# OpenPPL/ppq

Hardware: AMD Instinct MI355X
Metric: calibration samples/sec (RuntimeCalibrationPass, KL 2048-bin, ResNet-50 INT8) (higher is better)
Workload: dtype f32; 1 GPU; ResNet-50 topology (53 Conv + 1 Gemm, BN folded, seeded He init), RuntimeCalibrationPass kl 2048 bins, per-tensor INT8 activations, per-channel INT8 weights, 279 batches x 32 x 3x224x224 per GPU; samples=8928, batch=32, observed_tensors=72, rccl_ranks=1, async_observe=False, cache_params=False, channels_last=False, fuse_params=True, batch_observations=True, reuse_activations=False, replayed_batches=0, hip_graph=auto, graph_replays=0, miopen_find=False

## Files before the change

include/ppq_hip.h:

```cpp
#ifndef PPQ_HIP_H_
#define PPQ_HIP_H_

#include <stdint.h>

#ifdef __cplusplus
extern "C" {
#endif

typedef enum {
    PPQHIP_OK = 0,
    PPQHIP_ERR_INVALID_VALUE = -1,
    PPQHIP_ERR_UNSUPPORTED = -2,
    PPQHIP_ERR_HIP = -3
} ppqhip_status;

#define PPQHIP_ABI_VERSION 4

const char* ppqhip_last_error(void);
int ppqhip_version(void);
int ppqhip_device_arch(char* buf, int n);

int ppqhip_fq_linear_t(const float* x, const float* scale, const float* offset, float* out,
                       int64_t n, int clip_min, int clip_max, int rounding, void* stream);

// ... 368 lines not shown

enum { PPQHIP_MXFP8_E4M3 = 0, PPQHIP_MXFP8_E5M2 = 1, PPQHIP_MXFP6_E3M2 = 2, PPQHIP_MXFP6_E2M3 = 3, PPQHIP_MXFP4_E2M1 = 4,
       PPQHIP_MXINT8 = 5 };
int ppqhip_mx_fq(const float* x, float* y, uint8_t* scale_codes, int64_t outer, int64_t axis_len, int64_t inner, int format,
                 void* stream);
typedef struct ppqhip_mx_job {
    const float* x;
    float* y;
    uint8_t* scale_codes;
    int64_t outer, axis_len, inner;
    int32_t format, reserved;
} ppqhip_mx_job;
int ppqhip_mx_fq_multi(const ppqhip_mx_job* jobs, int num_jobs, void* stream);

int ppqhip_mx_pack(const float* x, uint8_t* elements, uint8_t* scales, int64_t outer, int64_t axis_len, int64_t inner, int format,
                   void* stream);
typedef struct ppqhip_mx_pack_job {
    const float* x;
    uint8_t* elements;
    uint8_t* scales;
    int64_t outer, axis_len, inner;
    int32_t format, reserved;
} ppqhip_mx_pack_job;
int ppqhip_mx_pack_multi(const ppqhip_mx_pack_job* jobs, int num_jobs, void* stream);
int ppqhip_mx_unpack(const uint8_t* elements, const uint8_t* scales, float* y, int64_t outer, int64_t axis_len, int64_t inner,
                     int format, void* stream);
typedef struct ppqhip_mx_unpack_job {
    const uint8_t* elements;
    const uint8_t* scales;
    float* y;
    int64_t outer, axis_len, inner;
    int32_t format, reserved;
} ppqhip_mx_unpack_job;
int ppqhip_mx_unpack_multi(const ppqhip_mx_unpack_job* jobs, int num_jobs, void* stream);

int ppqhip_mx_gemm(const uint8_t* a_elements, const uint8_t* a_scales, int a_format, const uint8_t* b_elements,
                   const uint8_t* b_scales, int b_format, const float* bias, float* c, int64_t m, int64_t n, int64_t k,
                   void* stream);

int ppqhip_mx_conv2d(const uint8_t* x_elements, const uint8_t* x_scales, int x_format, const uint8_t* w_elements,
                     const uint8_t* w_scales, int w_format, const float* bias, float* y, int64_t n, int64_t c, int64_t h, int64_t w,
                     int64_t o, int64_t kh, int64_t kw, int64_t stride_h, int64_t stride_w, int64_t pad_h, int64_t pad_w,
                     int64_t dil_h, int64_t dil_w, void* stream);

int ppqhip_mx_gemm_fused(const uint8_t* a_elements, const uint8_t* a_scales, int a_format, const uint8_t* b_elements,
                         const uint8_t* b_scales, int b_format, const float* bias, const float* residual, int relu, float* c,
                         uint8_t* out_elements, uint8_t* out_scales, int out_format, int64_t m, int64_t n, int64_t k, void* stream);
int ppqhip_mx_conv2d_fused(const uint8_t* x_elements, const uint8_t* x_scales, int x_format, const uint8_t* w_elements,
                           const uint8_t* w_scales, int w_format, const float* bias, const float* residual, int relu, float* y,
                           uint8_t* out_elements, uint8_t* out_scales, int out_format, int64_t n, int64_t c, int64_t h, int64_t w,
                           int64_t o, int64_t kh, int64_t kw, int64_t stride_h, int64_t stride_w, int64_t pad_h, int64_t pad_w,
                           int64_t dil_h, int64_t dil_w, void* stream);

#define PPQHIP_PROF_MAX_KERNELS 48
typedef struct {
    char name[48];
    int64_t launches;
    double total_ms;
    double total_bytes;
} ppqhip_prof_entry;
int ppqhip_prof_enable(int on);
int ppqhip_prof_collect(ppqhip_prof_entry* entries, int max_entries);
double ppqhip_prof_event_overhead_us(void* stream, int pairs);

#ifdef __cplusplus
}
#endif
#endif
```

ppq_amd/_lib.py:

```python
import ctypes
import os

_HERE = os.path.dirname(os.path.abspath(__file__))
LIB_PATH = os.path.join(_HERE, 'libppq_hip.so')

c_f32p = ctypes.c_void_p
c_i32p = ctypes.c_void_p
c_f64p = ctypes.c_void_p
c_i64 = ctypes.c_int64
c_int = ctypes.c_int
c_flt = ctypes.c_float
c_vp = ctypes.c_void_p

ABI_VERSION = 4


NOT_FUSED = 1


class ProfEntry(ctypes.Structure):
    _fields_ = [('name', ctypes.c_char * 48), ('launches', ctypes.c_int64),
                ('total_ms', ctypes.c_double), ('total_bytes', ctypes.c_double)]


# ... 55 lines not shown
    'ppqhip_fq_float_multi_table_bytes': (c_i64, [c_int]),
    'ppqhip_fq_float_multi': (c_int, [c_vp, c_int, c_int, c_vp, c_int, c_vp]),
    'ppqhip_quantile_multi_workspace_bytes': (c_i64, [c_int, c_i64]),
    'ppqhip_quantile_t_multi': (c_int, [c_vp, c_int, c_flt, c_vp, c_vp]),
    'ppqhip_quantile_debug_layout': (None, [c_vp]),
    'ppqhip_quantile_hot_layout': (None, [c_vp]),
    'ppqhip_minmax_t_slots_multi': (c_int, [c_vp, c_int, c_vp]),
    'ppqhip_hist_t_rows_multi': (c_int, [c_vp, c_int, c_int, c_int, c_i64, c_vp]),
    'ppqhip_channel_sum': (c_int, [c_f32p, c_i64, c_i64, c_i64, c_f64p, c_vp]),
    'ppqhip_hist_rows': (c_i64, []),
    'ppqhip_hist_sym_t_rows': (c_int, [c_f32p, c_i64, c_flt, c_int, c_i32p, c_i64, c_vp]),
    'ppqhip_hist_asym_t_rows': (c_int, [c_f32p, c_i64, c_flt, c_flt, c_int, c_i32p, c_i64, c_vp]),
    'ppqhip_hist_rows_finish': (c_int, [c_i32p, c_i64, c_i32p, c_vp]),
    'ppqhip_check_bin_rule': (c_int, [c_f32p, c_i64, c_flt, c_flt, c_int, c_vp, c_vp]),
    'ppqhip_minmax_slots': (c_i64, []),
    'ppqhip_minmax_t_slots': (c_int, [c_f32p, c_i64, c_f32p, c_vp]),
    'ppqhip_minmax_slots_finish': (c_int, [c_f32p, c_f32p, c_vp]),
    'ppqhip_mse_loss_host': (c_flt, [ctypes.POINTER(ctypes.c_int64), c_i64, c_int, c_int, c_int]),
    'ppqhip_mse_search_workspace_bytes': (c_i64, [c_i64]),
    'ppqhip_mse_search': (c_int, [c_i32p, c_i64, c_i64, c_f64p, c_f64p, c_int, c_int, c_int, c_i32p, c_vp, c_vp]),
    'ppqhip_kl_num_candidates': (c_i64, [c_i64, c_int]),
    'ppqhip_kl_losses': (c_int, [c_i32p, c_i64, c_i64, c_int, c_f64p, c_vp]),
    'ppqhip_tensor_clip_t': (c_int, [c_f32p, c_f32p, c_f32p, c_f32p, c_i64, c_vp]),
    'ppqhip_tensor_clip_c': (c_int, [c_f32p, c_f32p, c_f32p, c_f32p, c_i64, c_i64, c_i64, c_vp]),
    'ppqhip_rounding_loss': (c_int, [c_f32p, c_f32p, c_f32p, c_f32p, c_i64, c_i64, c_i64, c_int, c_int, c_int, c_vp]),
    'ppqhip_rounding_loss_bwd': (c_int, [c_f32p, c_f32p, c_f32p, c_f32p, c_f32p, c_i64, c_i64, c_i64, c_int, c_int,
                                         c_int, c_vp]),
    'ppqhip_adaround_fwd_multi': (c_int, [c_vp, c_int, c_vp]),
    'ppqhip_adaround_bwd_multi': (c_int, [c_vp, c_int, c_f32p, c_vp]),
    'ppqhip_roundtune_fwd_multi': (c_int, [c_vp, c_int, c_vp]),
    'ppqhip_equalize_scale_multi': (c_int, [c_vp, c_int, c_vp]),
    'ppqhip_equalize_apply_multi': (c_int, [c_vp, c_int, c_vp]),
    'ppqhip_split_plan_multi': (c_int, [c_vp, c_int, c_vp]),
    'ppqhip_split_apply_multi': (c_int, [c_vp, c_int, c_vp]),
    'ppqhip_ssd_scales_multi': (c_int, [c_vp, c_int, c_vp]),
    'ppqhip_ssd_apply_multi': (c_int, [c_vp, c_int, c_vp]),
    'ppqhip_fq_measure_rows_multi': (c_int, [c_vp, c_int, c_vp]),
    'ppqhip_fetch_rows_multi': (c_int, [c_vp, c_int, c_vp]),
    'ppqhip_measure_rows_multi': (c_int, [c_vp, c_int, c_vp]),
    'ppqhip_measure_finish_multi': (c_int, [c_vp, c_int, c_vp]),
    'ppqhip_stat_moments_multi': (c_int, [c_vp, c_int, c_vp]),
    'ppqhip_stat_shape_multi': (c_int, [c_vp, c_int, c_vp]),
    'ppqhip_mx_fq': (c_int, [c_f32p, c_f32p, c_vp, c_i64, c_i64, c_i64, c_int, c_vp]),
    'ppqhip_mx_fq_multi': (c_int, [c_vp, c_int, c_vp]),
    'ppqhip_mx_pack': (c_int, [c_f32p, c_vp, c_vp, c_i64, c_i64, c_i64, c_int, c_vp]),
    'ppqhip_mx_pack_multi': (c_int, [c_vp, c_int, c_vp]),
    'ppqhip_mx_unpack': (c_int, [c_vp, c_vp, c_f32p, c_i64, c_i64, c_i64, c_int, c_vp]),
    'ppqhip_mx_unpack_multi': (c_int, [c_vp, c_int, c_vp]),
    'ppqhip_mx_gemm': (c_int, [c_vp, c_vp, c_int, c_vp, c_vp, c_int, c_f32p, c_f32p, c_i64, c_i64, c_i64, c_vp]),
    'ppqhip_prof_enable': (c_int, [c_int]),
    'ppqhip_mx_conv2d': (c_int, [c_vp, c_vp, c_int, c_vp, c_vp, c_int, c_f32p, c_f32p] + [c_i64] * 13 + [c_vp]),
    'ppqhip_mx_gemm_fused': (c_int, [c_vp, c_vp, c_int, c_vp, c_vp, c_int, c_f32p, c_f32p, c_int, c_f32p, c_vp, c_vp, c_int, c_i64, c_i64, c_i64, c_vp]),
    'ppqhip_mx_conv2d_fused': (c_int, [c_vp, c_vp, c_int, c_vp, c_vp, c_int, c_f32p, c_f32p, c_int, c_f32p, c_vp, c_vp, c_int] + [c_i64] * 13 + [c_vp]),
    'ppqhip_prof_collect': (c_int, [ctypes.POINTER(ProfEntry), c_int]),
    'ppqhip_prof_event_overhead_us': (ctypes.c_double, [c_vp, c_int]),
}

if not os.path.exists(LIB_PATH):
    raise ImportError(
        f'{LIB_PATH} is missing: the HIP kernel library has not been built.  Run '
        '`python -c "import __graft_entry__ as g; g.build()"` or `make -C ppq_amd/csrc` (needs hipcc, '
        'targets gfx950).  ppq_amd has no CPU / PyTorch fallback by design.')

import torch

_torch_hip = os.path.join(os.path.dirname(torch.__file__), 'lib', 'libamdhip64.so')
if os.path.exists(_torch_hip):
    ctypes.CDLL(_torch_hip, mode=ctypes.RTLD_GLOBAL)

try:
    lib = ctypes.CDLL(LIB_PATH)
except OSError as e:
    raise ImportError(f'cannot load {LIB_PATH}: {e}') from e

for _name, (_res, _args) in PROTOTYPES.items():
    _fn = getattr(lib, _name)
    _fn.restype = _res
    _fn.argtypes = _args


if lib.ppqhip_version() != ABI_VERSION:
    raise ImportError(f'{LIB_PATH} has ABI version {lib.ppqhip_version()}, this package needs {ABI_VERSION}: rebuild it '
                      '(`make -C ppq_amd/csrc` or `python -c "import __graft_entry__ as g; g.build()"`)')


def last_error() -> str:
    msg = lib.ppqhip_last_error()
    return msg.decode('utf-8', 'replace') if msg else ''
```

ppq_amd/ffi.py:

```python
import math
import threading
import weakref
from typing import List

import numpy as np
import torch

from . import _lib
from ._lib import lib

_KERNEL_FAILURE = 'Kernel Failure, '


_raw_stream = torch._C._cuda_getCurrentRawStream
_get_device = torch._C._cuda_getDevice


def _stream() -> int:
    return _raw_stream(_get_device())


def _check(t: torch.Tensor, dtype: torch.dtype, name: str) -> None:
    if not isinstance(t, torch.Tensor):
        raise TypeError(f'{name}: expected a torch.Tensor, got {type(t)}')
# ... 124 lines not shown
_HIST_JOB = np.dtype([('x', '<u8'), ('rows', '<u8'), ('n', '<i8'), ('p0', '<f4'), ('p1', '<f4')])


def _epilogue_geometry(ts, bias_list):
    t0 = ts[0]
    if not isinstance(t0, torch.Tensor) or t0.dtype is not _F32 or not t0.is_cuda or t0.dim() != 4 or t0.numel() == 0:
        return None
    shape, strides, dev = t0.shape, t0.stride(), t0.device
    for t in ts[1:]:
        if not isinstance(t, torch.Tensor) or t.dtype is not _F32 or t.device != dev or t.shape != shape or t.stride() != strides:
            return None
    C = int(shape[1])
    for bias in bias_list:
        if (not isinstance(bias, torch.Tensor) or bias.dtype is not _F32 or bias.device != dev or bias.dim() != 1
                or bias.numel() != C or not bias.is_contiguous()):
            return None
    if t0.is_contiguous(): return C, int(shape[2]) * int(shape[3])
    if t0.is_contiguous(memory_format=torch.channels_last): return C, 1
    return None


def _pool_launch(y: torch.Tensor, geo, pool):
    k, s, p = (int(v) for v in pool)
    if geo is None or not y.is_contiguous() or k < 1 or s < 1 or p < 0: return None
    N, C, H, W = (int(v) for v in y.shape)
    if H + 2 * p < k or W + 2 * p < k: return None
    pooled = torch.empty((N, C, (H + 2 * p - k) // s + 1, (W + 2 * p - k) // s + 1), dtype=_F32, device=y.device)
    return pooled, (y.numel(), C, H, W), (k, s, p, 1, 0)


def bias_act_(y: torch.Tensor, bias: torch.Tensor, relu: bool, pool=None):
    geo = _epilogue_geometry([y], [bias])
    if pool is not None:
        args = _pool_launch(y, geo, pool)
        if args is None: return None
        with _DeviceOf(y):
            ok = _fused_or_raise(lib.ppqhip_bias_act_pool(y.data_ptr(), bias.data_ptr(), args[0].data_ptr(), *args[1],
                                                          1 if relu else 0, *args[2], _stream()))
        return args[0] if ok else None
    if geo is None: return False
    with _DeviceOf(y):
        _raise(lib.ppqhip_bias_act(y.data_ptr(), bias.data_ptr(), y.numel(), geo[0], geo[1], 1 if relu else 0, _stream()))
    return True


def bias_add_act(a: torch.Tensor, bias_a: torch.Tensor, b: torch.Tensor, bias_b, relu: bool):
    geo = _epilogue_geometry([a, b], [bias_a] if bias_b is None else [bias_a, bias_b])
    if geo is None or a.data_ptr() == b.data_ptr(): return None
    out = torch.empty_like(a)
    with _DeviceOf(a):
        _raise(lib.ppqhip_bias_add_act(a.data_ptr(), bias_a.data_ptr(), b.data_ptr(), 0 if bias_b is None else bias_b.data_ptr(),
                                       out.data_ptr(), a.numel(), geo[0], geo[1], 1 if relu else 0, _stream()))
    return out


def _sink_slots(job, dev) -> int:
    if job is None: return 0
    slots = job[1]
    if (job[0] != 'minmax' or slots.dtype is not _F32 or slots.device != dev or not slots.is_contiguous()
            or slots.numel() != 2 * lib.ppqhip_minmax_slots()): raise ValueError('no sink for this job')
    return slots.data_ptr()


def _fused_or_raise(status: int) -> bool:
    if status == _lib.NOT_FUSED: return False
    _raise(status)
    return True


def bias_act_stats_(y: torch.Tensor, bias: torch.Tensor, relu: bool, job, pool=None, store: bool = True):
    geo = _epilogue_geometry([y], [bias])
    if geo is None or job is None: return None if pool is not None else False
    try: slots = _sink_slots(job, y.device)
    except ValueError: return None if pool is not None else False
    if pool is not None:
        args = _pool_launch(y, geo, pool)
        if args is None: return None
        with _DeviceOf(y):
            ok = _fused_or_raise(lib.ppqhip_bias_act_pool_stats(y.data_ptr(), bias.data_ptr(), args[0].data_ptr(), *args[1],
                                                                1 if relu else 0, *args[2], slots, 1 if store else 0, _stream()))
        return args[0] if ok else None
    with _DeviceOf(y):
        return _fused_or_raise(lib.ppqhip_bias_act_stats(y.data_ptr(), bias.data_ptr(), y.numel(), geo[0], geo[1],
                                                         1 if relu else 0, slots, _stream()))


ELIDE_A, ELIDE_B = 1, 2


def bias_add_act_stats(a: torch.Tensor, bias_a: torch.Tensor, b: torch.Tensor, bias_b, relu: bool, job_a, job_b, job_out,
                       elide: int = 0):
    geo = _epilogue_geometry([a, b], [bias_a] if bias_b is None else [bias_a, bias_b])
    if geo is None or a.data_ptr() == b.data_ptr(): return None
    if bias_b is None and job_b is not None: return None
    try: slots = [_sink_slots(j, a.device) for j in (job_a, job_b, job_out)]
    except ValueError: return None
    if not any(slots): return None
    out = torch.empty_like(a)
    args = (a.data_ptr(), bias_a.data_ptr(), b.data_ptr(), 0 if bias_b is None else bias_b.data_ptr(), out.data_ptr(),
            a.numel(), geo[0], geo[1], 1 if relu else 0, slots[0], slots[1], slots[2])
    with _DeviceOf(a):
        if elide: ok = _fused_or_raise(lib.ppqhip_bias_add_act_stats2(*args, int(elide), _stream()))
        else: ok = _fused_or_raise(lib.ppqhip_bias_add_act_stats(*args, _stream()))
    return out if ok else None


# ... 1778 lines not shown
```

ppq_amd/harness.py:

```python
import contextlib
from typing import Callable, Dict, List, Optional

import torch
import torch.nn.functional as F

from .core import LinearQuantizationConfig, QuantizationStates, TensorQuantizationConfig, is_initial
from .core import QuantizationProperty as P
from .qfunction import PPQuantFunction

PASSIVE_OPERATIONS = {'MaxPool', 'GlobalMaxPool', 'Reshape', 'Flatten', 'Identity', 'Dropout', 'Slice', 'Pad', 'Resize',
                      'Split', 'Transpose', 'Interp', 'Squeeze', 'Unsqueeze'}
COMPUTING_OP = {'Conv', 'Gemm', 'ConvTranspose', 'MatMul'}


class Variable:
    def __init__(self, name: str, value: torch.Tensor = None, is_parameter: bool = False):
        self.name = name
        self.value = value
        self.stored_value = None
        self.is_parameter = is_parameter
        self.dest_ops: List['Operation'] = []
        self.source_op: Optional['Operation'] = None

    def __hash__(self): return hash(self.name)
# ... 43 lines not shown
        return list(zip(self.config.input_quantization_config, self.inputs)) + \
            list(zip(self.config.output_quantization_config, self.outputs))

    def dequantize(self):
        if getattr(self, '_dequantized', False): return self
        for cfg, _ in self.config_with_variable:
            cfg.detail['Stored State'] = cfg.state
            cfg.state = QuantizationStates.FP32
        self._swap_parameters()
        self._dequantized = True
        return self

    def restore_quantize_state(self):
        if not getattr(self, '_dequantized', False): return self
        for cfg, _ in self.config_with_variable:
            if 'Stored State' in cfg.detail: cfg.state = cfg.detail.pop('Stored State')
        self._swap_parameters()
        self._dequantized = False
        return self

    def baking_parameters(self, quant_func: Callable):
        for config, var in self.config_with_variable:
            if var.is_parameter and QuantizationStates.is_activated(config.state):
                var.value = quant_func(var.value, config)
                config.state = (QuantizationStates.BAKED if config.state == QuantizationStates.ACTIVATED
                                else QuantizationStates.PASSIVE_BAKED)


class BaseGraph:
    def __init__(self, name: str):
        self.name = name
        self.operations: Dict[str, Operation] = {}
        self.variables: Dict[str, Variable] = {}
        self.inputs: Dict[str, Variable] = {}
        self.outputs: Dict[str, Variable] = {}

    def create_variable(self, name: str, value=None, is_parameter=False) -> Variable:
        v = Variable(name, value, is_parameter)
        self.variables[name] = v
        return v

    def create_operation(self, op_type: str, name: str, inputs: List[Variable], attributes: dict = None) -> Variable:
        out = self.create_variable(name + '_out')
        op = Operation(name, op_type, attributes, list(inputs), [out])
        out.source_op = op
        for v in inputs: v.dest_ops.append(op)
        self.operations[name] = op
        return out

    def topological_sort(self) -> List[Operation]:
        return list(self.operations.values())


def _forward(op: Operation, x: List[torch.Tensor]):
    t, a = op.type, op.attributes
    if t == 'Conv':
        return F.conv2d(x[0], x[1], x[2] if len(x) > 2 else None, stride=a.get('strides', 1),
                        padding=a.get('pads', 0), groups=a.get('group', 1))
    if t == 'Gemm': return F.linear(x[0], x[1], x[2] if len(x) > 2 else None)
    if t == 'MatMul': return torch.matmul(x[0], x[1])
    if t == 'Relu': return F.relu(x[0])
    if t == 'Gelu': return F.gelu(x[0])
    if t == 'Add': return x[0] + x[1]
    if t == 'MaxPool': return F.max_pool2d(x[0], a['kernel_shape'], a.get('strides', 1), a.get('pads', 0))
    if t == 'GlobalAveragePool': return F.adaptive_avg_pool2d(x[0], 1)
    if t == 'Flatten': return torch.flatten(x[0], 1)
    if t == 'LayerNormalization': return F.layer_norm(x[0], x[0].shape[-1:], x[1], x[2])
    if t == 'Softmax': return F.softmax(x[0], dim=a.get('axis', -1))
    if t == 'Mul': return x[0] * (x[1] if len(x) > 1 else a['value'])
    if t == 'Reshape': return x[0].reshape(a['shape'])
    if t == 'Transpose': return x[0].permute(a['perm'])
    if t == 'Concat': return torch.cat([v.expand(x[-1].shape[0], *v.shape[1:]) if v.shape[0] == 1 else v for v in x],
                                       dim=a.get('axis', 1))
    if t == 'Slice': return x[0].narrow(a['axis'], a['start'], a['length'])
    if t == 'Resize': return F.interpolate(x[0], scale_factor=a.get('scale', 2), mode=a.get('mode', 'nearest'))
    raise NotImplementedError(f'Graph op: {op.name}({op.type}) has no backend implementation')


class EpilogueGroup:
    __slots__ = ('kind', 'ops', 'convs', 'add', 'relu', 'keep', 'pool')

    def __init__(self, kind, ops, convs, add, relu, keep=(), pool=None):
        self.kind, self.ops, self.convs, self.add, self.relu, self.keep = kind, ops, convs, add, relu, frozenset(keep)
        self.pool = pool

    def __repr__(self): return f'{self.kind}({", ".join(op.name for op in self.ops)})'


def pool_window(op: Operation) -> Optional[tuple]:
    a = op.attributes

    def square(value):
        if isinstance(value, (list, tuple)):
            if not 1 <= len(value) <= 2 or any(v != value[0] for v in value): return None
            value = value[0]
        return value if isinstance(value, int) and not isinstance(value, bool) else None
    if 'kernel_shape' not in a or square(a.get('dilations', 1)) != 1 or a.get('ceil_mode', 0) not in (0, False): return None
    window = tuple(square(v) for v in (a['kernel_shape'], a.get('strides', 1), a.get('pads', 0)))
    return None if any(v is None for v in window) else window


def _in_cfg(op, i):
    return op.config.input_quantization_config[i] if isinstance(op, QuantableOperation) else None


def _out_cfg(op, i):
    return op.config.output_quantization_config[i] if isinstance(op, QuantableOperation) else None


def plan_epilogues(operations: List[Operation], hooks: Dict[str, object] = None, keep=(), passes_through: Callable = None,
                   grad_enabled: bool = False) -> List[EpilogueGroup]:
# ... 70 lines not shown
        return EpilogueGroup('P1', [conv, relu] + ([pool] if pool is not None else []), [conv], None, relu, keep, pool)

    groups, i = [], 0
    while i < len(operations):
        g = try_p2(i) if operations[i].type == 'Conv' else None
        if g is None and operations[i].type == 'Conv': g = try_p1(i)
        if g is None:
            i += 1
            continue
        groups.append(g)
        i += len(g.ops)
    return groups


def elidable_stores(grp: EpilogueGroup, hooks, jobs: Dict[str, tuple], recorder=None) -> set:
    if recorder is not None or not hooks: return set()
    if grp.kind == 'P2': producers, reader = grp.convs, grp.add
    elif grp.pool is not None: producers, reader = [grp.relu], grp.pool
    else: return set()
    reader_hook = hooks.get(reader.name)
    out = set()
    for op in producers:
        v, hook = op.outputs[0], hooks.get(op.name)
        if len(v.dest_ops) != 1 or v.dest_ops[0] is not reader or v.name in grp.keep: continue
        if op.name not in jobs or hook is None or not isinstance(op, QuantableOperation): continue
        obs = [hook._observer_table.get(c) for c in op.config.output_quantization_config]
        if len(obs) != 1 or obs[0] is None or not obs[0].reads_only_its_job(): continue
        if reader_hook is not None and isinstance(reader, QuantableOperation) and any(
                c in reader_hook._observer_table for x, c in zip(reader.inputs, reader.config.input_quantization_config) if x is v):
            continue
        out.add(op.name)
    return out


class TorchExecutor:
    def __init__(self, graph: BaseGraph, device: str = 'cuda'):
        self._graph = graph
        self._device = device
        self._default_quant_fn = PPQuantFunction
        self.cache_parameter_quantization = False
        self._param_cache: Dict[str, tuple] = {}
        self.fuse_parameter_quantization = True
        self._plans: list = []
        self._plan_signature = None
        self._plan_cache: Dict[tuple, list] = {}
        self._fused: Dict[tuple, torch.Tensor] = {}
        self._delegates: Dict[object, Callable] = {}
        self._overrides: Dict[str, Callable] = {}
        self._takes_packed: set = set()
        self._group_overrides: Dict[str, tuple] = {}
        self.fuse_epilogues = True
        self._epilogue_cache: Dict[tuple, dict] = {}
        self.channels_last = False
        for v in graph.variables.values():
            if v.is_parameter and v.value is not None: v.value = v.value.to(device)

    def use_channels_last(self) -> 'TorchExecutor':
        self.channels_last = True
        for v in self._graph.variables.values():
            if v.is_parameter and isinstance(v.value, torch.Tensor) and v.value.dim() == 4:
                v.value = v.value.contiguous(memory_format=torch.channels_last)
        return self

    def _place(self, value: torch.Tensor) -> torch.Tensor:
        value = value.to(self._device)
        if self.channels_last and value.dim() == 4: value = value.contiguous(memory_format=torch.channels_last)
        return value

    def register_quantize_delegate(self, config, delegator: Callable) -> None:
        self._delegates[config] = delegator

    def remove_quantize_delegate(self, config) -> None:
        self._delegates.pop(config, None)

    def register_operation_override(self, op_name: str, fn: Callable, takes_packed: bool = False) -> None:
        if op_name not in self._graph.operations: raise KeyError(f'register_operation_override: the graph has no operation {op_name!r}')
        if not callable(fn): raise TypeError(f'register_operation_override: fn must be callable, got {type(fn)}')
        self._overrides[op_name] = fn
        if takes_packed: self._takes_packed.add(op_name)
        else: self._takes_packed.discard(op_name)

    def remove_operation_override(self, op_name: str) -> None:
        self._overrides.pop(op_name, None)
        self._takes_packed.discard(op_name)

    def register_group_override(self, op_names: List[str], fn: Callable) -> None:
        if not op_names: raise ValueError('register_group_override: no operations')
        for name in op_names:
            if name not in self._graph.operations: raise KeyError(f'register_group_override: the graph has no operation {name!r}')
        if not callable(fn): raise TypeError(f'register_group_override: fn must be callable, got {type(fn)}')
        self._group_overrides[op_names[0]] = (tuple(op_names), fn)

    def remove_group_override(self, first_name: str) -> None:
        self._group_overrides.pop(first_name, None)

    def _group_plan(self, operations: List[Operation], hooks, output_names, all_float: bool) -> Dict[str, tuple]:
        if not self._group_overrides: return {}
        hooks = hooks or {}
        keep = set(self._graph.outputs) | set(output_names or ())
        at = {op.name: i for i, op in enumerate(operations)}
        plan = {}
        for first, (names, fn) in self._group_overrides.items():
            if any(n not in at or n in hooks for n in names): continue
            if any(at[a] >= at[b] for a, b in zip(names, names[1:])): continue
            ops = [operations[at[n]] for n in names]
            if any(v.name in keep for m in ops[:-1] for v in m.outputs): continue
            need = set()
            for v in ops[-1].outputs:
                handed = [d.name in self._takes_packed and d.name in self._overrides and d.name not in hooks and d.name in at
                          and d.inputs[0] is v and sum(1 for x in d.inputs if x is v) == 1 for d in v.dest_ops]
                if all_float or v.name in keep or not handed or not all(handed): need.add(v.name)
            plan[first] = (ops, fn, need)
        return plan

    def _run_group(self, entry: tuple, raw_of: Callable, packed: Dict[str, object]) -> Dict[str, object]:
        ops, fn, need = entry
        inside = {v.name for m in ops for v in m.outputs}
        inputs = [[None if v.name in inside else raw_of(v) for v in m.inputs] for m in ops]
        head = ops[0]
        if head.name in self._takes_packed and head.inputs[0].name in packed: inputs[0][0] = packed[head.inputs[0].name]
        if any(x is None for k, m in enumerate(ops) for x, v in zip(inputs[k], m.inputs) if v.name not in inside):
            raise ValueError(f'group override of {head.name}: an input was not computed')
        values, handed = fn(ops, inputs, need)
        out = {}
        for m in ops:
            for v in m.outputs:
                if v.name in values: out[v.name] = values[v.name]
                elif v.name in handed and v.name not in need: out[v.name] = handed[v.name]
                else: raise RuntimeError(f'group override of {head.name}: no {"float " if v.name in need else ""}value for {v.name}')
        packed.update(handed)
        return out

    def _override_inputs(self, op: Operation, raw_in: list, packed: Dict[str, object]) -> list:
        if packed and op.name in self._takes_packed and op.inputs[0].name in packed:
            raw_in = list(raw_in)
            raw_in[0] = packed[op.inputs[0].name]
        return raw_in

    def quantize_function(self, tensor: torch.Tensor, config=None) -> torch.Tensor:
        if self._delegates and config in self._delegates:
            return self._delegates[config](tensor, config)
        return self._default_quant_fn(tensor, config)

    def _input_side(self, op: Operation, raw_in: list, hook) -> list:
        qin, cfgs = raw_in, None
        if isinstance(op, QuantableOperation):
            cfgs = list(op.config.input_quantization_config)
            qin = [self._quantize_parameter(v, c) if v.is_parameter else self.quantize_function(x, c)
                   for v, x, c in zip(op.inputs, raw_in, cfgs)]
        if hook is not None: qin = hook.pre_forward_hook(inputs=raw_in, quant_inputs=qin, quant_configs=cfgs)
        return qin

    def _output_side(self, op: Operation, outs, hook) -> list:
        fp_outs = outs = list(outs) if isinstance(outs, (list, tuple)) else [outs]
        cfgs = None
        if isinstance(op, QuantableOperation):
            cfgs = list(op.config.output_quantization_config)
            outs = [self.quantize_function(y, c) for y, c in zip(outs, cfgs)]
        if hook is not None: outs = hook.post_forward_hook(outputs=fp_outs, quant_outputs=outs, quant_configs=cfgs)
        return outs

    def _step(self, op: Operation, raw_in: list, hook, packed: Optional[Dict[str, object]]) -> list:
        override = self._overrides.get(op.name) if hook is None else None
        if override is not None: outs = override(op, self._override_inputs(op, raw_in, packed))
        else: outs = _forward(op, self._input_side(op, raw_in, hook))
        return self._output_side(op, outs, hook)

    def _walk(self, operations: List[Operation], hooks, output_names: List[str], read: Callable, write: Callable,
              hand_packed: bool = False, write_aliases: bool = True, done: Callable = None, unfed: str = None) -> None:
        groups, packed = self._group_plan(operations, hooks, output_names, not hand_packed), {}
        plan = self._epilogue_plan(operations, hooks, output_names, [m.name for e in groups.values() for m in e[0]])
        fused_done = set()
        for op in operations:
            if op.name in fused_done: continue
            vals = None
            if op.name in groups:
                members = groups[op.name][0]
                vals, aliases = self._run_group(groups[op.name], read, packed), members[:-1]
            elif op.name in plan:
                grp = plan[op.name]
                vals, members, aliases = self._run_epilogue(grp, read, hooks), grp.ops, (grp.add or grp.convs[0],)
            if vals is None:
                raw_in = [read(v) for v in op.inputs]
                if unfed and any(x is None for x in raw_in): raise ValueError(f'{unfed}: input of {op.name} was not fed')
                write(op, self._step(op, raw_in, hooks.get(op.name) if hooks else None, packed if hand_packed else None))
            else:
                for m in members:
                    fused_done.add(m.name)
                    if write_aliases or m not in aliases: write(m, [vals[v.name] for v in m.outputs])
            if done is not None and done(): break

    def forward_with_gradient(self, inputs, output_names: List[str] = None, hooks=None):
        return TorchExecutor.forward.__wrapped__(self, inputs, output_names, hooks)

    def partial_graph_forward(self, operations: List[Operation], feed_dict: Dict[str, torch.Tensor],
                              output_names: List[str], with_gradient: bool = False) -> List[torch.Tensor]:
        g = self._graph
        results = [None] * len(output_names)

        def write(op, outs):
            for v, y in zip(op.outputs, outs):
                v.value = y
                if v.name in output_names: results[output_names.index(v.name)] = y
        with contextlib.nullcontext() if with_gradient else torch.no_grad():
            for name, value in feed_dict.items(): g.variables[name].value = self._place(value)
            self._fused_parameters(operations)
            self._walk(operations, None, output_names, lambda v: v.value, write, unfed='partial_graph_forward')
        for v in g.variables.values():
            if not v.is_parameter: v.value = None
        return results

    def _fused_parameters(self, operations=None) -> None:
        self._fused = {}
        if not self.fuse_parameter_quantization or self._default_quant_fn is not PPQuantFunction: return
        from .ffi import FloatingQuantizePlan, LinearQuantizePlan
        todo, sig = [], []
        for op in (self._graph.operations.values() if operations is None else operations):
            if not isinstance(op, QuantableOperation): continue
# ... 27 lines not shown
                if floating:
                    plan = FloatingQuantizePlan([(v.value, c.scale, c.offset, axis, c.exponent_bits, c.mantissa_bits,
                                                  c.quant_min, c.quant_max) for v, c, axis, _, _ in items], rounding=rnd)
                else:
                    plan = LinearQuantizePlan([(v.value, c.scale, c.offset, axis, c.quant_min, c.quant_max)
                                               for v, c, axis, _, _ in items], rounding=rnd)
                self._plans.append((plan, [(v.name, id(c)) for v, c, _, _, _ in items]))
            self._plan_signature = sig
            if len(self._plan_cache) >= 8: self._plan_cache.pop(next(iter(self._plan_cache)))
            self._plan_cache[tuple(sig)] = self._plans
        for plan, keys in self._plans:
            for key, out in zip(keys, plan.run()): self._fused[key] = out

    def _epilogue_plan(self, operations: List[Operation], hooks, output_names, grouped=()) -> Dict[str, EpilogueGroup]:
        if not self.fuse_epilogues or torch.is_grad_enabled() or self._default_quant_fn is not PPQuantFunction: return {}
        states = tuple(c.state for op in operations if isinstance(op, QuantableOperation)
                       for c in (*op.config.input_quantization_config, *op.config.output_quantization_config))
        sig = (tuple(op.name for op in operations), tuple((k, id(h)) for k, h in hooks.items()) if hooks else (),
               tuple(output_names or ()), tuple(id(c) for c in self._delegates), states, tuple(sorted(self._overrides)), tuple(sorted(grouped)))
        plan = self._epilogue_cache.get(sig)
        if plan is None:
            delegates = self._delegates

            def passes_through(c): return not QuantizationStates.is_activated(c.state) and c not in delegates
            groups = plan_epilogues(operations, hooks, set(self._graph.outputs) | set(output_names or ()), passes_through)
            if self._overrides:
                groups = [g for g in groups if not any(m.name in self._overrides and not (hooks and m.name in hooks) for m in g.ops)]
            if grouped:
                groups = [g for g in groups if not any(m.name in grouped for m in g.ops)]
            plan = {g.ops[0].name: g for g in groups}
            if len(self._epilogue_cache) >= 8: self._epilogue_cache.pop(next(iter(self._epilogue_cache)))
            self._epilogue_cache[sig] = plan
        return plan

    def _run_epilogue(self, grp: EpilogueGroup, raw_of: Callable, hooks) -> Optional[Dict[str, torch.Tensor]]:
        from .ffi import (ELIDE_A, ELIDE_B, bias_act_, bias_act_hist_, bias_act_stats_, bias_add_act, bias_add_act_hist,
                          bias_add_act_stats)
        for conv in grp.convs:
            x, w = raw_of(conv.inputs[0]), conv.inputs[1].value
            if not (isinstance(x, torch.Tensor) and x.is_cuda and x.dtype == torch.float32 and x.dim() == 4
                    and isinstance(w, torch.Tensor) and w.dim() == 4): return None
            fmt = torch.channels_last if self.channels_last else torch.contiguous_format
            if not (x.is_contiguous(memory_format=fmt) and w.is_contiguous(memory_format=fmt)): return None
        if grp.add is not None:
            b_var = grp.add.inputs[1]
            if b_var.source_op not in grp.convs:
                b = raw_of(b_var)
                if not (isinstance(b, torch.Tensor) and b.is_cuda and b.dtype == torch.float32): return None
        hooks = hooks or {}
        ys, biases = {}, {}
        for conv in grp.ops[:len(grp.convs)]:
            qin = self._input_side(conv, [raw_of(v) for v in conv.inputs], hooks.get(conv.name))
            a = conv.attributes
            ys[conv.name] = F.conv2d(qin[0], qin[1], None, stride=a.get('strides', 1), padding=a.get('pads', 0),
                                     groups=a.get('group', 1))
            biases[conv.name] = qin[2]
        if grp.kind == 'P1':
            conv = grp.convs[0]
            y = ys[conv.name]
            stored = {grp.relu.name: y}
            fed = self._epilogue_sinks(grp, hooks, stored, y)
            window = pool_window(grp.pool) if grp.pool is not None and not self.channels_last else None
            pooled, elided = None, set()
            if fed is not None:
                job = fed[0].get(grp.relu.name)
                launch = bias_act_hist_ if job is not None and job[0] == 'hist_rows' else bias_act_stats_
                if window is not None:
                    elided = elidable_stores(grp, hooks, fed[0], fed[1].recorder)
                    pooled = launch(y, biases[conv.name], True, job, pool=window, store=not elided)
                    if pooled is None: elided = set()
                if pooled is None and not launch(y, biases[conv.name], True, job): fed = None
            if fed is None:
                if window is not None: pooled = bias_act_(y, biases[conv.name], relu=True, pool=window)
                if pooled is None and not bias_act_(y, biases[conv.name], relu=True):
                    y.add_(biases[conv.name].view(1, -1, 1, 1)).relu_()
            tail = {conv.name: y, grp.relu.name: y}
            if grp.pool is not None: tail[grp.pool.name] = pooled
        else:
            conv_a = grp.convs[0]
            a = ys[conv_a.name]
            conv_b = grp.convs[1] if len(grp.convs) > 1 else None
            b = ys[conv_b.name] if conv_b is not None else raw_of(grp.add.inputs[1])
            bias_b = biases[conv_b.name] if conv_b is not None else None
            stored = {conv_a.name: a, grp.relu.name: None}
            if conv_b is not None: stored[conv_b.name] = b
            fed, out, elided = self._epilogue_sinks(grp, hooks, stored, a), None, set()
            if fed is not None:
                jobs = fed[0]
                elided = elidable_stores(grp, hooks, jobs, fed[1].recorder)
                mask = (ELIDE_A if conv_a.name in elided else 0) | (ELIDE_B if conv_b is not None and conv_b.name in elided else 0)
                launch = bias_add_act_hist if next(iter(jobs.values()))[0] == 'hist_rows' else bias_add_act_stats
                out = launch(a, biases[conv_a.name], b, bias_b, True, jobs.get(conv_a.name),
                             jobs.get(conv_b.name) if conv_b is not None else None, jobs.get(grp.relu.name), mask)
                if out is None: fed, elided = None, set()
                else: stored[grp.relu.name] = out
            if out is None: out = bias_add_act(a, biases[conv_a.name], b, bias_b, relu=True)
            if out is None:
                a.add_(biases[conv_a.name].view(1, -1, 1, 1))
                if conv_b is not None: b.add_(biases[conv_b.name].view(1, -1, 1, 1))
                out = F.relu(a + b)
            tail = {conv_a.name: a, grp.add.name: out, grp.relu.name: out}
            if conv_b is not None: tail[conv_b.name] = b
        if fed is not None:
            for name, job in fed[0].items(): fed[1].prepay(stored[name], job[1])
        values: Dict[str, torch.Tensor] = {}
        for op in grp.ops:
            hook = hooks.get(op.name)
            if op.type != 'Conv':
# ... 374 lines not shown
```

Before: 3858 samples/s.

## Add native MFMA 1x1 conv kernel and route selected pointwise convs to it

```diff
diff --git a/include/ppq_hip.h b/include/ppq_hip.h
--- a/include/ppq_hip.h
+++ b/include/ppq_hip.h
@@ -444,6 +444,9 @@
                            int64_t o, int64_t kh, int64_t kw, int64_t stride_h, int64_t stride_w, int64_t pad_h, int64_t pad_w,
                            int64_t dil_h, int64_t dil_w, void* stream);
 
+int ppqhip_conv1x1(const float* x, const float* w, const float* bias, float* y, int64_t n, int64_t c, int64_t h, int64_t wd,
+                   int64_t o, int64_t stride, void* stream);
+
 #define PPQHIP_PROF_MAX_KERNELS 48
 typedef struct {
     char name[48];
diff --git a/ppq_amd/_lib.py b/ppq_amd/_lib.py
--- a/ppq_amd/_lib.py
+++ b/ppq_amd/_lib.py
@@ -131,7 +131,8 @@
     'ppqhip_mx_conv2d': (c_int, [c_vp, c_vp, c_int, c_vp, c_vp, c_int, c_f32p, c_f32p] + [c_i64] * 13 + [c_vp]),
     'ppqhip_mx_gemm_fused': (c_int, [c_vp, c_vp, c_int, c_vp, c_vp, c_int, c_f32p, c_f32p, c_int, c_f32p, c_vp, c_vp, c_int, c_i64, c_i64, c_i64, c_vp]),
     'ppqhip_mx_conv2d_fused': (c_int, [c_vp, c_vp, c_int, c_vp, c_vp, c_int, c_f32p, c_f32p, c_int, c_f32p, c_vp, c_vp, c_int] + [c_i64] * 13 + [c_vp]),
-    'ppqhip_prof_collect': (c_int, [ctypes.POINTER(ProfEntry), c_int]),
+    'ppqhip_conv1x1': (c_int, [c_f32p, c_f32p, c_f32p, c_f32p, c_i64, c_i64, c_i64, c_i64, c_i64, c_i64, c_vp]),
+    'ppqhip_prof_collect':(c_int, [ctypes.POINTER(ProfEntry), c_int]),
     'ppqhip_prof_event_overhead_us': (ctypes.c_double, [c_vp, c_int]),
 }
 
diff --git a/ppq_amd/csrc/pointwise_conv.hip b/ppq_amd/csrc/pointwise_conv.hip
--- /dev/null
+++ b/ppq_amd/csrc/pointwise_conv.hip
@@ -0,0 +1,194 @@
+#include "common.hpp"
+#include "job_table.hpp"
+
+namespace ppqhip {
+namespace {
+
+typedef float f32x16 __attribute__((ext_vector_type(16)));
+
+struct PwArgs {
+    const float* x; const float* w; const float* bias; float* y;
+    uint32_t c, o, q;
+    uint32_t in_plane, out_plane;
+    uint32_t in_w, stride;
+    uint32_t tiles_m;
+    FastDiv div_plane, div_wo, div_tiles_m;
+};
+
+template <int WM, int WN, int TM, int TN, int BK, bool VEC>
+__global__ __launch_bounds__(256) void conv1x1_kernel(const PwArgs g) {
+    static_assert(WM * WN == 4 && (BK == 16 || BK == 32), "4 waves; BK 16 or 32");
+    constexpr int BM = WM * TM * 32, BN = WN * TN * 32, RS = BK + 4, HK = BK / 2, LW = VEC ? 4 : 1;
+    constexpr int WL = BM * BK / (256 * LW), XL = BK * BN / (256 * LW);
+    constexpr int WROWS = 256 * LW / BK, XROWS = 256 * LW / BN;
+    static_assert(BN / LW <= 256 && WL >= 1 && XL >= 1, "tile too small / too wide for the loader");
+    typedef float ldv __attribute__((ext_vector_type(LW)));
+    __shared__ __attribute__((aligned(16))) float Ws[2][BM * RS];
+    __shared__ __attribute__((aligned(16))) float Xs[2][BK * BN];
+
+    const uint32_t t = threadIdx.x, lane = t & 63u, wave = t >> 6;
+    const uint32_t tq = fdiv(blockIdx.x, g.div_tiles_m), tm = blockIdx.x - tq * g.tiles_m;
+    const uint32_t m0 = tm * BM, q0 = tq * BN;
+
+    const uint32_t wk = (t % (BK / LW)) * LW, wm = t / (BK / LW);
+    const uint32_t xc = (t % (BN / LW)) * LW, xk = t / (BN / LW);
+    uint32_t woff[WL], xoff;
+#pragma unroll
+    for (int r = 0; r < WL; r++) woff[r] = min(m0 + wm + WROWS * r, g.o - 1u) * g.c + wk;
+    {
+        const uint32_t qx = min(q0 + xc, g.q - LW);
+        const uint32_t img = fdiv(qx, g.div_plane), p = qx - img * g.out_plane;
+        uint32_t src = p;
+        if (g.stride != 1u) { const uint32_t oh = fdiv(p, g.div_wo), ow = p - oh * g.div_wo.d; src = (oh * g.in_w + ow) * g.stride; }
+        xoff = img * g.c * g.in_plane + src + xk * g.in_plane;
+    }
+    const uint32_t xstep = XROWS * g.in_plane;
+    ldv wr[WL], xr[XL];
+    auto load_tile = [&](uint32_t k0) {
+        if (k0 + BK <= g.c) {
+#pragma unroll
+            for (int r = 0; r < WL; r++) wr[r] = *reinterpret_cast<const ldv*>(g.w + (woff[r] + k0));
+            const float* xp = g.x + (xoff + k0 * g.in_plane);
+#pragma unroll
+            for (int r = 0; r < XL; r++) xr[r] = *reinterpret_cast<const ldv*>(xp + r * xstep);
+        } else {
+#pragma unroll
+            for (int r = 0; r < WL; r++) {
+                ldv pad = -0.0f;
+                wr[r] = (k0 + wk < g.c) ? *reinterpret_cast<const ldv*>(g.w + (woff[r] + k0)) : pad;
+            }
+#pragma unroll
+            for (int r = 0; r < XL; r++) {
+                ldv pad = 0.0f;
+                xr[r] = (k0 + xk + XROWS * r < g.c) ? *reinterpret_cast<const ldv*>(g.x + (xoff + k0 * g.in_plane + r * xstep)) : pad;
+            }
+        }
+    };
+    auto store_tile = [&](int buf) {
+#pragma unroll
+        for (int r = 0; r < WL; r++) {
+            float* row = &Ws[buf][(wm + WROWS * r) * RS];
+            if constexpr (VEC) {
+                *reinterpret_cast<float2*>(row + (wk >> 1)) = make_float2(wr[r][0], wr[r][2]);
+                *reinterpret_cast<float2*>(row + HK + (wk >> 1)) = make_float2(wr[r][1], wr[r][3]);
+            } else {
+                row[(wk & 1u) * HK + (wk >> 1)] = wr[r][0];
+            }
+        }
+#pragma unroll
+        for (int r = 0; r < XL; r++) *reinterpret_cast<ldv*>(&Xs[buf][(xk + XROWS * r) * BN + xc]) = xr[r];
+    };
+
+    const uint32_t i = lane & 31u, h = lane >> 5;
+    const uint32_t row0 = (wave / WN) * (TM * 32), col0 = (wave % WN) * (TN * 32);
+    f32x16 acc[TM][TN];
+#pragma unroll
+    for (int mt = 0; mt < TM; mt++)
+#pragma unroll
+        for (int nt = 0; nt < TN; nt++)
+#pragma unroll
+            for (int r = 0; r < 16; r++) acc[mt][nt][r] = 0.0f;
+
+    const uint32_t tiles_k = (g.c + BK - 1) / BK;
+    load_tile(0);
+    store_tile(0);
+    __syncthreads();
+    for (uint32_t kt = 0; kt < tiles_k; kt++) {
+        const int buf = (int)(kt & 1u);
+        const bool more = kt + 1 < tiles_k;
+        if (more) load_tile((kt + 1) * BK);
+        const float* ws = &Ws[buf][(row0 + i) * RS + h * HK];
+        const float* xs = &Xs[buf][h * BN + col0 + i];
+        float a[TM][HK];
+#pragma unroll
+        for (int mt = 0; mt < TM; mt++)
+#pragma unroll
+            for (int v = 0; v < HK / 4; v++) {
+                const float4 f = *reinterpret_cast<const float4*>(ws + mt * 32 * RS + 4 * v);
+                a[mt][4 * v] = f.x; a[mt][4 * v + 1] = f.y; a[mt][4 * v + 2] = f.z; a[mt][4 * v + 3] = f.w;
+            }
+#pragma unroll
+        for (int s = 0; s < HK; s++) {
+            float b[TN];
+#pragma unroll
+            for (int nt = 0; nt < TN; nt++) b[nt] = xs[2 * s * BN + nt * 32];
+#pragma unroll
+            for (int mt = 0; mt < TM; mt++)
+#pragma unroll
+                for (int nt = 0; nt < TN; nt++)
+                    acc[mt][nt] = __builtin_amdgcn_mfma_f32_32x32x2f32(a[mt][s], b[nt], acc[mt][nt], 0, 0, 0);
+        }
+        if (more) store_tile(buf ^ 1);
+        __syncthreads();
+    }
+
+    const bool has_bias = g.bias != nullptr;
+    float bv[TM][16];
+#pragma unroll
+    for (int mt = 0; mt < TM; mt++)
+#pragma unroll
+        for (int r = 0; r < 16; r++)
+            bv[mt][r] = has_bias ? g.bias[min(m0 + row0 + mt * 32 + (r & 3) + 8 * (r >> 2) + 4 * h, g.o - 1u)] : 0.0f;
+#pragma unroll
+    for (int nt = 0; nt < TN; nt++) {
+        const uint32_t qc = q0 + col0 + nt * 32 + i;
+        if (qc >= g.q) continue;
+        const uint32_t img = fdiv(qc, g.div_plane), p = qc - img * g.out_plane;
+        float* yc = g.y + (img * g.o * g.out_plane + p);
+#pragma unroll
+        for (int mt = 0; mt < TM; mt++)
+#pragma unroll
+            for (int r = 0; r < 16; r++) {
+                const uint32_t row = m0 + row0 + mt * 32 + (r & 3) + 8 * (r >> 2) + 4 * h;
+                if (row >= g.o) continue;
+                float v = acc[mt][nt][r];
+                if (has_bias) v = v + bv[mt][r];
+                yc[row * g.out_plane] = v;
+            }
+    }
+}
+
+constexpr int kWM = 2, kWN = 2, kTM = 1, kTN = 1, kBK = 32;
+
+inline bool aligned4(const void* p) { return (reinterpret_cast<uintptr_t>(p) & 3u) == 0; }
+
+}
+}
+
+using namespace ppqhip;
+
+extern "C" int ppqhip_conv1x1(const float* x, const float* w, const float* bias, float* y, int64_t n, int64_t c, int64_t h, int64_t wd,
+                              int64_t o, int64_t stride, void* stream) {
+    const char* what = "conv1x1";
+    constexpr int64_t kMax = 2147483647;
+    if (n < 0 || c <= 0 || h <= 0 || wd <= 0 || o <= 0) { set_error("%s: non-positive size", what); return PPQHIP_ERR_INVALID_VALUE; }
+    if (stride != 1 && stride != 2) { set_error("%s: stride must be 1 or 2", what); return PPQHIP_ERR_UNSUPPORTED; }
+    if (n == 0) return PPQHIP_OK;
+    if (x == nullptr || w == nullptr || y == nullptr) { set_error("%s: null pointer", what); return PPQHIP_ERR_INVALID_VALUE; }
+    const int64_t ho = (h - 1) / stride + 1, wo = (wd - 1) / stride + 1;
+    if (n > kMax || c > kMax || h > kMax || wd > kMax || o > kMax || (double)n * (double)c * (double)h * (double)wd > (double)kMax
+        || (double)n * (double)o * (double)ho * (double)wo > (double)kMax || (double)o * (double)c > (double)kMax) {
+        set_error("%s: more than 2^31 - 1 elements in x, w or y", what); return PPQHIP_ERR_INVALID_VALUE;
+    }
+    std::vector<Span> ins, outs;
+    ins.push_back(span_of(x, n * c * h * wd)); ins.push_back(span_of(w, o * c));
+    if (bias != nullptr) ins.push_back(span_of(bias, o));
+    outs.push_back(span_of(y, n * o * ho * wo));
+    if (int st = check_overlap(what, ins, outs)) return st;
+    if (!aligned4(x) || !aligned4(w) || !aligned4(y) || !aligned4(bias)) return PPQHIP_NOT_FUSED;
+
+    PwArgs g;
+    g.x = x; g.w = w; g.bias = bias; g.y = y;
+    g.c = (uint32_t)c; g.o = (uint32_t)o; g.q = (uint32_t)(n * ho * wo);
+    g.in_plane = (uint32_t)(h * wd); g.out_plane = (uint32_t)(ho * wo); g.in_w = (uint32_t)wd; g.stride = (uint32_t)stride;
+    g.div_plane = make_fastdiv(g.out_plane); g.div_wo = make_fastdiv((uint32_t)wo);
+    hipStream_t s = (hipStream_t)stream;
+    const bool vec = stride == 1 && g.out_plane % 4u == 0 && c % 4 == 0 && aligned16(x) && aligned16(w);
+    constexpr uint32_t BM = kWM * kTM * 32, BN = kWN * kTN * 32;
+    g.tiles_m = (g.o + BM - 1) / BM;
+    g.div_tiles_m = make_fastdiv(g.tiles_m);
+    const dim3 grid(g.tiles_m * ((g.q + BN - 1) / BN));
+    if (vec) hipLaunchKernelGGL((conv1x1_kernel<kWM, kWN, kTM, kTN, kBK, true>), grid, dim3(256), 0, s, g);
+    else hipLaunchKernelGGL((conv1x1_kernel<kWM, kWN, kTM, kTN, kBK, false>), grid, dim3(256), 0, s, g);
+    return finish_launch(what);
+}
diff --git a/ppq_amd/ffi.py b/ppq_amd/ffi.py
--- a/ppq_amd/ffi.py
+++ b/ppq_amd/ffi.py
@@ -200,6 +200,25 @@
         _raise(lib.ppqhip_bias_add_act(a.data_ptr(), bias_a.data_ptr(), b.data_ptr(), 0 if bias_b is None else bias_b.data_ptr(),
                                        out.data_ptr(), a.numel(), geo[0], geo[1], 1 if relu else 0, _stream()))
     return out
+
+
+def conv1x1(x: torch.Tensor, w: torch.Tensor, bias, stride: int = 1):
+    _f32(x, 'x'); _f32(w, 'w')
+    if x.dim() != 4 or not x.is_contiguous() or not w.is_contiguous() or w.dim() not in (2, 4) or w.numel() != w.shape[0] * w.shape[1]:
+        raise RuntimeError(_KERNEL_FAILURE + 'conv1x1: x must be contiguous NCHW and w a contiguous [O, C, 1, 1] or [O, C]')
+    N, C, H, W = (int(v) for v in x.shape)
+    O = int(w.shape[0])
+    if int(w.shape[1]) != C or w.device != x.device: raise RuntimeError(_KERNEL_FAILURE + 'conv1x1: w does not match x')
+    if bias is not None:
+        _f32(bias, 'bias')
+        if bias.dim() != 1 or bias.numel() != O or not bias.is_contiguous() or bias.device != x.device:
+            raise RuntimeError(_KERNEL_FAILURE + 'conv1x1: bias must be a contiguous [O] vector on the device of x')
+    stride = int(stride)
+    y = torch.empty((N, O, (H - 1) // max(stride, 1) + 1, (W - 1) // max(stride, 1) + 1), dtype=_F32, device=x.device)
+    with _DeviceOf(x):
+        ok = _fused_or_raise(lib.ppqhip_conv1x1(x.data_ptr(), w.data_ptr(), 0 if bias is None else bias.data_ptr(), y.data_ptr(),
+                                                N, C, H, W, O, stride, _stream()))
+    return y if ok else None
 
 
 def _sink_slots(job, dev) -> int:
diff --git a/ppq_amd/harness.py b/ppq_amd/harness.py
--- a/ppq_amd/harness.py
+++ b/ppq_amd/harness.py
@@ -119,11 +119,46 @@
         return list(self.operations.values())
 
 
-def _forward(op: Operation, x: List[torch.Tensor]):
+POINTWISE_MIN_WORK = 3.2e9
+POINTWISE_KEEP_VENDOR = frozenset({
+    (64, 64, 56, 56, 1), (64, 256, 56, 56, 1), (256, 64, 56, 56, 1), (256, 128, 56, 56, 1), (128, 512, 28, 28, 1),
+    (512, 256, 28, 28, 1), (1024, 256, 14, 14, 1), (1024, 512, 14, 14, 1), (512, 2048, 7, 7, 1), (1024, 2048, 14, 14, 2),
+    (2048, 512, 7, 7, 1)})
+
+
+def _square(v):
+    if isinstance(v, (list, tuple)):
+        return int(v[0]) if len(v) > 0 and all(int(e) == int(v[0]) for e in v) else None
+    return int(v)
+
+
+def pointwise_eligible(x, w, attributes: dict, min_work: float) -> bool:
+    a = attributes or {}
+    if not (isinstance(x, torch.Tensor) and isinstance(w, torch.Tensor) and x.dim() == 4 and w.dim() == 4): return False
+    if tuple(w.shape[2:]) != (1, 1) or w.shape[1] != x.shape[1]: return False
+    if _square(a.get('pads', 0)) != 0 or _square(a.get('dilations', 1)) != 1 or a.get('group', 1) != 1: return False
+    stride = _square(a.get('strides', 1))
+    if stride not in (1, 2): return False
+    if not (x.is_cuda and w.is_cuda and x.dtype is torch.float32 and w.dtype is torch.float32): return False
+    if not (x.is_contiguous() and w.is_contiguous()) or x.numel() == 0: return False
+    if torch.is_grad_enabled() or x.requires_grad or w.requires_grad: return False
+    n, c, h, wd = (int(v) for v in x.shape)
+    o = int(w.shape[0])
+    if (c, o, h, wd, stride) in POINTWISE_KEEP_VENDOR: return False
+    return 2.0 * n * o * c * ((h - 1) // stride + 1) * ((wd - 1) // stride + 1) >= min_work
+
+
+def _conv(x, w, bias, a: dict, native_min_work=None):
+    if native_min_work is not None and pointwise_eligible(x, w, a, native_min_work):
+        from .ffi import conv1x1
+        y = conv1x1(x, w, bias, _square(a.get('strides', 1)))
+        if y is not None: return y
+    return F.conv2d(x, w, bias, stride=a.get('strides', 1), padding=a.get('pads', 0), groups=a.get('group', 1))
+
+
+def _forward(op: Operation, x: List[torch.Tensor], native_min_work=None):
     t, a = op.type, op.attributes
-    if t == 'Conv':
-        return F.conv2d(x[0], x[1], x[2] if len(x) > 2 else None, stride=a.get('strides', 1),
-                        padding=a.get('pads', 0), groups=a.get('group', 1))
+    if t == 'Conv': return _conv(x[0], x[1], x[2] if len(x) > 2 else None, a, native_min_work)
     if t == 'Gemm': return F.linear(x[0], x[1], x[2] if len(x) > 2 else None)
     if t == 'MatMul': return torch.matmul(x[0], x[1])
     if t == 'Relu': return F.relu(x[0])
@@ -300,6 +335,8 @@
         self.fuse_epilogues = True
         self._epilogue_cache: Dict[tuple, dict] = {}
         self.channels_last = False
+        self.native_pointwise_conv = True
+        self.pointwise_min_work = POINTWISE_MIN_WORK
         for v in graph.variables.values():
             if v.is_parameter and v.value is not None: v.value = v.value.to(device)
 
@@ -309,6 +346,9 @@
             if v.is_parameter and isinstance(v.value, torch.Tensor) and v.value.dim() == 4:
                 v.value = v.value.contiguous(memory_format=torch.channels_last)
         return self
+
+    def _native_min_work(self):
+        return self.pointwise_min_work if self.native_pointwise_conv and not self.channels_last else None
 
     def _place(self, value: torch.Tensor) -> torch.Tensor:
         value = value.to(self._device)
@@ -411,7 +451,10 @@
     def _step(self, op: Operation, raw_in: list, hook, packed: Optional[Dict[str, object]]) -> list:
         override = self._overrides.get(op.name) if hook is None else None
         if override is not None: outs = override(op, self._override_inputs(op, raw_in, packed))
-        else: outs = _forward(op, self._input_side(op, raw_in, hook))
+        else:
+            qin, native = self._input_side(op, raw_in, hook), self._native_min_work()
+            if native is not None and op.type == 'Conv' and pointwise_eligible(qin[0], qin[1], op.attributes, native): outs = _forward(op, qin, native)
+            else: outs = _forward(op, qin)
         return self._output_side(op, outs, hook)
 
     def _walk(self, operations: List[Operation], hooks, output_names: List[str], read: Callable, write: Callable,
@@ -545,8 +588,7 @@
         for conv in grp.ops[:len(grp.convs)]:
             qin = self._input_side(conv, [raw_of(v) for v in conv.inputs], hooks.get(conv.name))
             a = conv.attributes
-            ys[conv.name] = F.conv2d(qin[0], qin[1], None, stride=a.get('strides', 1), padding=a.get('pads', 0),
-                                     groups=a.get('group', 1))
+            ys[conv.name] = _conv(qin[0], qin[1], None, a, self._native_min_work())
             biases[conv.name] = qin[2]
         if grp.kind == 'P1':
             conv = grp.convs[0]
```

Result: faster. 3901 samples/s (median of 6 runs) (+1.1%).
